# OSU-Bee-Lab/buzzdetect

Measured on AMD Instinct MI355X. Metric: yamnet_windows_per_s, higher is better.
Workload: dtype f32 (split-f16x3 MFMA products, f32 accumulate)

## Files before the change

buzzdetect_amd/csrc/bd_internal.h:

```cpp
#pragma once

#include <hip/hip_runtime.h>
#include <stdint.h>

#include <vector>

#include "../../include/buzzdetect_hip.h"

namespace bd {

constexpr int kMelNonZero = 461;

constexpr int kMelStart[BD_MEL_BANDS] = {
    5, 5, 6, 7, 9, 10, 11, 12, 13, 14, 16, 17, 18, 20, 21, 23, 25, 26, 28, 30, 32, 34, 36, 38, 40, 42, 44, 47, 49, 52, 54, 57,
    60, 63, 66, 69, 72, 76, 79, 83, 87, 90, 95, 99, 103, 108, 112, 117, 122, 127, 133, 138, 144, 150, 156, 162, 169, 176, 183,
    190, 198, 206, 214, 223};
constexpr int kMelLen[BD_MEL_BANDS] = {
    1, 2, 3, 3, 2, 2, 2, 2, 3, 3, 2, 3, 3, 3, 4, 3, 3, 4, 4, 4, 4, 4, 4, 4, 4, 5, 5, 5, 5, 5, 6, 6,
    6, 6, 6, 7, 7, 7, 8, 7, 8, 9, 8, 9, 9, 9, 10, 10, 11, 11, 11, 12, 12, 12, 13, 14, 14, 14, 15, 16, 16, 17, 17, 17};
constexpr int mel_offset(int band) {
    int o = 0;
    for (int m = 0; m < band; ++m) o += kMelLen[m];
    return o;
}
// ... 100 lines not shown
bool launch_l4_reg_f32(const float* in, float* out, int windows, const SepLayer& L4, const SepLayer& L5, hipStream_t stream);
bool launch_separable_chip(const float* in, float* out, int windows, const SepLayer* L, int nl, hipStream_t stream,
                           const SepLayer* next = nullptr, bool planes = false);
bool tail_supported(const SepLayer& L13, const SepLayer& L14);
bool launch_tail_pw13_dw14(const void* in, void* out, int windows, const SepLayer& L13, const SepLayer& L14, hipStream_t stream);
bool launch_tail_pw14_pool(const void* in, float* pooled, int windows, const SepLayer& L14, hipStream_t stream);
bool tail_f32_supported(const SepLayer& L13, const SepLayer& L14);
bool launch_tail_f32(const float* in, float* mid, float* pooled, int windows, const SepLayer& L13, const SepLayer& L14, hipStream_t stream,
                     int which);
bool launch_separable_chip_f32(const float* in, float* out, int windows, const SepLayer* L, int nl, hipStream_t stream,
                               const SepLayer* next, bool dw0_done);
bool launch_separable_mid_f32(const float* in, float* out, int windows, const SepLayer& L5, const SepLayer& L6, const SepLayer& L7,
                              hipStream_t stream);
bool launch_separable_mid(const float* in, float* out, int windows, const SepLayer& L5, const SepLayer& L6, const SepLayer& L7,
                          hipStream_t stream);
int launch_separable_run_next_dw(const float* a, float* b, int windows, const SepLayer* L, int max_layers, hipStream_t stream,
                                 bool planes = false);
bool launch_separable_fused_next_dw(const float* in, float* out, int windows, const SepLayer& L, const SepLayer& next,
                                    hipStream_t stream);
bool l4_window_planes_supported(const SepLayer& L3, const SepLayer& L4, const SepLayer& L5);
bool launch_l4_window_planes(const void* planes, const SepLayer& L3, const SepLayer& L4, const SepLayer& L5, float* out,
                             int windows, hipStream_t stream);
void launch_stem_reg(const float* logmel, int patch_step, const WindowMap& map, int w0, int windows, const float* c1_w,
                     const float* c1_b, const SepLayer& L2, const SepLayer& L3, float* out, hipStream_t stream);
void launch_stem_reg_planes(const float* logmel, int patch_step, const WindowMap& map, int w0, int windows, const float* c1_w,
                            const float* c1_b, const SepLayer& L2, const SepLayer& L3, float* out, hipStream_t stream);
void launch_stem_reg_f32(const float* logmel, int patch_step, const WindowMap& map, int w0, int windows, const float* c1_w,
                         const float* c1_b, const SepLayer& L2, const SepLayer& L3, float* out, hipStream_t stream);
void launch_stem4(const float* logmel, int patch_step, const WindowMap& map, int w0, int windows, const float* c1_w,
                  const float* c1_b,
// ... 8 lines not shown
```

buzzdetect_amd/csrc/engine.hip:

```cpp
#include <cmath>
#include <cstdio>
#include <cstdlib>
#include <cstring>
#include <unistd.h>
#include <memory>
#include <string>
#include <type_traits>
#include <utility>
#include <vector>

#include "bd_internal.h"

namespace {

thread_local std::string g_error;

int fail(int code, const std::string& msg) {
    g_error = msg;
    return code;
}

#define BD_HIP(expr)                                                                            \
    do {                                                                                        \
        hipError_t e_ = (expr);                                                                 \
        if (e_ != hipSuccess)                                                                   \
            return fail(BD_EHIP, std::string(#expr) + ": " + hipGetErrorString(e_));            \
    } while (0)

const int kLayerDefs[14][2] = {{2, 32},  {1, 64},  {2, 128}, {1, 128}, {2, 256}, {1, 256},  {2, 512},
                               {1, 512}, {1, 512}, {1, 512}, {1, 512}, {1, 512}, {2, 1024}, {1, 1024}};

constexpr int64_t kFloatsA = 98304;
constexpr int64_t kFloatsB = 49152;
constexpr int kDefaultGroup = 1024;
constexpr int kMaxGroup = 65536;
static_assert(kMaxGroup <= 1 << 17, "the tail launchers of pass_f16 / pass_f32 cover the largest pass");

inline int64_t align_up(int64_t v, int64_t a) { return (v + a - 1) / a * a; }

struct Event2 {
    hipEvent_t ev;
    int slot;
};

}

struct bd_engine {
    int device = 0;
    int n_classes = 0;
    int group_windows = kDefaultGroup;
    int pointwise_mode = 1;
// ... 808 lines not shown
    if (e->stem == 3 && e->separable != 0 && bd::l4_window_planes_supported(sep[1], sep[2], sep[3])) {
        stem(g, bd::launch_stem_reg_planes);
        if (!g.launch(7, [&] { return bd::launch_l4_window_planes(g.a, sep[1], sep[2], sep[3], g.b, g.gw, g.stream); }))
            return fail(BD_EHIP, "l4_window_kernel declined the planes of the stem");
    } else {
        if (e->stem != 0) {
            stem(g, e->stem == 3 ? bd::launch_stem_reg : bd::launch_stem4);
        } else {
            conv1(g);
            walk_layers(g, 0, false, 4);
        }
        if (e->separable == 0) return walk_layers(g, 2, false, -1);
        if (!g.launch(7, [&] { return bd::launch_separable_fused_next_dw(g.a, g.b, g.gw, sep[2], sep[3], g.stream); }))
            return walk_layers(g, 2, false, -1);
    }
    if (!(e->separable == 1 &&
          g.launch(13, [&] { return bd::launch_separable_mid(g.b, g.a, g.gw, sep[3], sep[4], sep[5], g.stream); }))) {
        pointwise(g, 3);
        if (!g.launch(11, [&] { return bd::launch_separable_fused_next_dw(g.a, g.b, g.gw, sep[4], sep[5], g.stream); }))
            return walk_layers(g, 4, false, -1);
        pointwise(g, 5);
    }
    const bool planes = bd::tail_supported(sep[11], sep[12]);
    if (!g.launch(23, [&] { return bd::launch_separable_run_next_dw(g.a, g.b, g.gw, &sep[6], 7, g.stream, planes); }))
        return walk_layers(g, 6, false, -1);
    if (!planes) return walk_layers(g, 11, true, -1);
    float* const pooled = g.emb ? g.emb : g.b;
    if (!g.launch(25, [&] { return bd::launch_tail_pw13_dw14(g.b, g.a, g.gw, sep[11], sep[12], g.stream); }) ||
        !g.launch(27, [&] { return bd::launch_tail_pw14_pool(g.a, pooled, g.gw, sep[12], g.stream); }))
        return fail(BD_EHIP, "septail.hip declined the planes of the on-chip run");
    return head(g, pooled);
}

int pass_f32(Group& g) {
    const bd_engine* e = g.e;
    const bd::SepLayer* sep = g.sep;
    stem(g, bd::launch_stem_reg_f32);
    if (e->separable == 0) return walk_layers(g, 2, false, -1);
    if (!g.launch(7, [&] { return bd::launch_l4_reg_f32(g.a, g.b, g.gw, sep[2], sep[3], g.stream); }))
        return walk_layers(g, 2, false, -1);
    bool dw8_done = false;
// ... 505 lines not shown
```

buzzdetect_amd/csrc/sepchip.hip:

```cpp
#include "bd_internal.h"

#include <cstdio>
#include <cstdlib>
#include <mutex>

namespace bd {

namespace {

typedef float f32x16 __attribute__((ext_vector_type(16)));
typedef float v2f __attribute__((ext_vector_type(2)));
typedef _Float16 f16x8 __attribute__((ext_vector_type(8)));

constexpr float kF16MaxChip = 65504.0f;

constexpr int kChipHalfBytes = 97 * 64;
constexpr int kChipSlotBytes = 2 * kChipHalfBytes;

constexpr int kChipMaxLayers = 5;
struct ChipChain {
    const float* dw_w[kChipMaxLayers];
    const float* dw_b[kChipMaxLayers];
    const _Float16* whi[kChipMaxLayers];
    const _Float16* wlo[kChipMaxLayers];
    const float* pw_u[kChipMaxLayers];
    const float* pw_b[kChipMaxLayers];
    const float* ndw_w;
};
template <typename T>
__device__ __forceinline__ const T* chain_ptr(int field, int li) {
    typedef const __attribute__((address_space(4))) unsigned long long* kptr;
    const kptr ka = (kptr)__builtin_amdgcn_kernarg_segment_ptr();
    return reinterpret_cast<const T*>(ka[field * kChipMaxLayers + li]);
}
static_assert(sizeof(ChipChain) == (6 * kChipMaxLayers + 1) * 8, "six tables of five pointers + one");

template <bool PLAIN, int NSLOT, bool TRACE = false, bool NDW = false, bool PLANES = false>
__global__ __launch_bounds__(512, 2) void sep_chip_kernel(const ChipChain ch, const float* X, float* Y, int nl,
                                                           long long M, unsigned* __restrict__ range_flag,
                                                           unsigned long long* __restrict__ dbg = nullptr, int tune = 0) {
    static_assert(NSLOT >= 9 && NSLOT <= 16, "ring size");
    constexpr int K = 512, KQ = K / 16;
    constexpr int NPEND = 16 - NSLOT;
    extern __shared__ __attribute__((aligned(16))) char sm[];
    const int tid = threadIdx.x;
    const int lane = tid & 63;
    const int wc = __builtin_amdgcn_readfirstlane(tid >> 6);
    const int frow = lane & 31, fh = lane >> 5;
    const long long m0 = (long long)blockIdx.x * 96;
    float rmax = 0.0f;
    int tsn = 0;
#define CHIP_TS()                                                                                         \
// ... 47 lines not shown
        char* const slot0 = sm + wc * kChipSlotBytes;                                                     \
        _Pragma("unroll") for (int rl = 0; rl < 48; ++rl) CHIP_PUT(slot0, rl, out0[rl])                   \
        if (wc + 8 < NSLOT) {                                                \
            char* const slot1 = sm + (wc + 8) * kChipSlotBytes;                                           \
            _Pragma("unroll") for (int rl = 0; rl < 48; ++rl) CHIP_PUT(slot1, rl, pend[rl])               \
        }                                                                                                 \
    }
#define CHIP_PUT(SLOT, RL, PK)                                                                            \
    {                                                                                                     \
        char* const p_ = (SLOT) + (wbl ^ ((((RL) >> 2) & 3) << 4)) + (RL) * 64;                           \
        *reinterpret_cast<unsigned short*>(p_) = (unsigned short)(PK);                                    \
        *reinterpret_cast<unsigned short*>(p_ + kChipHalfBytes) = (unsigned short)((PK) >> 16);           \
    }
#define CHIP_TAPS_RSRC(DW_W) __builtin_amdgcn_make_buffer_rsrc(const_cast<float*>(DW_W), 0, 10 * K * 4, 0x00020000)

    const long long rows_left = M - m0;
    const unsigned tile_bytes = (unsigned)(rows_left < 96 ? rows_left : 96) * (K * 4);
    {
        const __amdgpu_buffer_rsrc_t xrs = __builtin_amdgcn_make_buffer_rsrc(const_cast<float*>(X) + (size_t)m0 * K, 0, tile_bytes, 0x00020000);
        const __amdgpu_buffer_rsrc_t taps0 = CHIP_TAPS_RSRC(ch.dw_w[0]);
        const unsigned xo = (48u * fh * K) * 4 + c4;
#pragma unroll
        for (int j = 0; j < 2; ++j) {
            const int st = j ? wc + 8 : wc;
            v2f in2[6][4];
#pragma unroll
            for (int y = 0; y < 6; ++y)
#pragma unroll
                for (int x = 0; x < 4; ++x) {
                    in2[y][x].x = __builtin_bit_cast(float, __builtin_amdgcn_raw_buffer_load_b32(xrs, xo, ((4 * y + x) * K + 32 * st) * 4, 0));
                    in2[y][x].y = __builtin_bit_cast(float, __builtin_amdgcn_raw_buffer_load_b32(xrs, xo, ((24 + 4 * y + x) * K + 32 * st) * 4, 0));
                }
            if (j == 0) CHIP_DW(0, st, taps0)
            else CHIP_DW(1, st, taps0)
            CHIP_TS()
            __builtin_amdgcn_sched_barrier(0);
        }
        CHIP_PUBLISH()
    }

    for (int li = 0; li < nl; ++li) {
        const _Float16* const Wfhi = chain_ptr<_Float16>(2, li);
        const _Float16* const Wflo = chain_ptr<_Float16>(3, li);
        const __amdgpu_buffer_rsrc_t bhr = __builtin_amdgcn_make_buffer_rsrc(const_cast<_Float16*>(Wfhi), 0, K * K * 2, 0x00020000);
        const __amdgpu_buffer_rsrc_t blr = __builtin_amdgcn_make_buffer_rsrc(const_cast<_Float16*>(Wflo), 0, K * K * 2, 0x00020000);
        const int btile = wc * (KQ * 1024);
        constexpr int jstep = 8 * KQ * 1024;
        f16x8 bh0[2], bl0[2], bh1[2], bl1[2];
#define CHIP_LB(R, B, Q, J) B[J] = __builtin_bit_cast(f16x8, __builtin_amdgcn_raw_buffer_load_b128(R, lane16, btile + (J) * jstep + (Q) * 1024, 0));
#define CHIP_BLOAD(BH, BL, Q) { CHIP_LB(bhr, BH, Q, 0) CHIP_LB(blr, BL, Q, 0) CHIP_LB(bhr, BH, Q, 1) CHIP_LB(blr, BL, Q, 1) }
        CHIP_BLOAD(bh0, bl0, 0)
        __syncthreads();
        CHIP_TS()

        float zero;
        asm volatile("v_mov_b32 %0, 0" : "=v"(zero));
#pragma unroll
        for (int i = 0; i < 3; ++i)
#pragma unroll
            for (int j = 0; j < 2; ++j)
#pragma unroll
                for (int r = 0; r < 16; ++r) acc[i][j][r] = zero;
// ... 11 lines not shown
    }                                                                                                     \
    CHIP_MF(I, 0, AH, BH[0]) M3 CHIP_SB                                                                   \
    if constexpr (!PLAIN) {                                                                               \
        CHIP_MF(I, 1, AL, BH[1]) M4 CHIP_SB                                                               \
        CHIP_MF(I, 1, AH, BL[1]) M5 CHIP_SB                                                               \
    } else {                                                                                              \
        M4 M5                                                                                             \
    }                                                                                                     \
    CHIP_MF(I, 1, AH, BH[1]) M6 CHIP_SB
#define CHIP_STAGES(FROM, TO)                                                                             \
    if ((FROM) < (TO)) {                                                                                  \
        f16x8 ah0, al0, ah1, al1, ah2, al2;                                                               \
        const char* abase = sm + ((FROM) < NSLOT ? (FROM) : (FROM) - NSLOT) * kChipSlotBytes;             \
        CHIP_LAH(ah0, 0, 0) CHIP_LAL(al0, 0, 0) CHIP_LAH(ah1, 0, 1) CHIP_LAL(al1, 0, 1)                   \
        _Pragma("nounroll") for (int kk = (FROM); kk < (TO); ++kk) {                                      \
            const int q1 = 2 * kk + 1, q2 = 2 * kk + 2 < KQ ? 2 * kk + 2 : 0;      \
            const char* const anext = sm + (kk + 1 < (TO) ? (kk + 1 < NSLOT ? kk + 1 : kk + 1 - NSLOT) : (kk < NSLOT ? kk : kk - NSLOT)) * kChipSlotBytes; \
            CHIP_STEP(0, ah0, al0, bh0, bl0, CHIP_LB(bhr, bh1, q1, 0), CHIP_LB(blr, bl1, q1, 0), CHIP_LB(bhr, bh1, q1, 1),  \
                      CHIP_LB(blr, bl1, q1, 1), CHIP_LAH(ah2, 0, 2), CHIP_LAL(al2, 0, 2))                 \
            CHIP_STEP(1, ah1, al1, bh0, bl0, CHIP_LAH(ah0, 1, 0), CHIP_LAL(al0, 1, 0), CHIP_NOP, CHIP_NOP, CHIP_NOP, CHIP_NOP) \
            CHIP_STEP(2, ah2, al2, bh0, bl0, CHIP_LAH(ah1, 1, 1), CHIP_LAL(al1, 1, 1), CHIP_LB(blr, bl0, q2, 0),            \
                      CHIP_LB(bhr, bh0, q2, 0), CHIP_NOP, CHIP_LB(blr, bl0, q2, 1))                       \
            CHIP_STEP(0, ah0, al0, bh1, bl1, CHIP_LB(bhr, bh0, q2, 1), CHIP_LAH(ah2, 1, 2), CHIP_LAL(al2, 1, 2), CHIP_NOP, CHIP_NOP, CHIP_NOP) \
            abase = anext;          \
            CHIP_STEP(1, ah1, al1, bh1, bl1, CHIP_LAH(ah0, 0, 0), CHIP_LAL(al0, 0, 0), CHIP_NOP, CHIP_NOP, CHIP_NOP, CHIP_NOP) \
            CHIP_STEP(2, ah2, al2, bh1, bl1, CHIP_LAH(ah1, 0, 1), CHIP_LAL(al1, 0, 1), CHIP_NOP, CHIP_NOP, CHIP_NOP, CHIP_NOP) \
        }                                                                                                 \
    }
        CHIP_STAGES(0, NPEND)
        CHIP_TS()
        if constexpr (NPEND > 0) {
            __syncthreads();
            CHIP_TS()
            if (wc >= 8 - NPEND) {
                char* const slot = sm + (wc + 8 - NSLOT) * kChipSlotBytes;
                int wbl = wb0;
                asm volatile("" : "+v"(wbl));
#pragma unroll
                for (int rl = 0; rl < 48; ++rl) CHIP_PUT(slot, rl, pend[rl])
            }
        }
        CHIP_TS()
        if constexpr (NPEND > 0) __syncthreads();
        CHIP_TS()
        CHIP_STAGES(NPEND, 16)
        CHIP_TS()
#undef CHIP_STAGES
#undef CHIP_STEP
#undef CHIP_BLOAD
#undef CHIP_LB
#undef CHIP_LAH
#undef CHIP_LAL
#undef CHIP_MF
#undef CHIP_SB
#undef CHIP_NOP
        if (li + 1 == nl) break;

        const __amdgpu_buffer_rsrc_t taps = CHIP_TAPS_RSRC(chain_ptr<float>(0, li + 1));
        const __amdgpu_buffer_rsrc_t pur = __builtin_amdgcn_make_buffer_rsrc(const_cast<float*>(chain_ptr<float>(4, li)), 0, K * 4, 0x00020000);
        const __amdgpu_buffer_rsrc_t pbr = __builtin_amdgcn_make_buffer_rsrc(const_cast<float*>(chain_ptr<float>(5, li)), 0, K * 4, 0x00020000);
#pragma unroll
        for (int j = 0; j < 2; ++j) {
            const int st = j ? wc + 8 : wc;
            const float u = __builtin_bit_cast(float, __builtin_amdgcn_raw_buffer_load_b32(pur, c4, 128 * st, 0));
            const float b = __builtin_bit_cast(float, __builtin_amdgcn_raw_buffer_load_b32(pbr, c4, 128 * st, 0));
            float ev[12][4];
#pragma unroll
            for (int q = 0; q < 6; ++q)
#pragma unroll
                for (int x = 0; x < 4; ++x) {
                    const float a01 = fmaxf(fmaf(acc[q >> 2][j][4 * (q & 3) + x], u, b), 0.0f);
                    const float a23 = fmaxf(fmaf(acc[(q + 6) >> 2][j][4 * ((q + 6) & 3) + x], u, b), 0.0f);
                    const auto r = __builtin_amdgcn_permlane32_swap(__builtin_bit_cast(unsigned, a01),
                                                                    __builtin_bit_cast(unsigned, a23), false, false);
                    ev[2 * q][x] = __builtin_bit_cast(float, (unsigned)r[0]);
                    ev[2 * q + 1][x] = __builtin_bit_cast(float, (unsigned)r[1]);
                }
            v2f in2[6][4];
#pragma unroll
            for (int y = 0; y < 6; ++y)
#pragma unroll
                for (int x = 0; x < 4; ++x) in2[y][x] = v2f{ev[y][x], ev[6 + y][x]};
            if (j == 0) CHIP_DW(0, st, taps)
            else CHIP_DW(1, st, taps)
            CHIP_TS()
        }
        __syncthreads();
        CHIP_TS()
        CHIP_PUBLISH()
    }
#undef CHIP_DW
#undef CHIP_PUBLISH
#undef CHIP_TAPS_RSRC
#undef CHIP_PUT

    {
        const __amdgpu_buffer_rsrc_t pur = __builtin_amdgcn_make_buffer_rsrc(const_cast<float*>(chain_ptr<float>(4, nl - 1)), 0, K * 4, 0x00020000);
        const __amdgpu_buffer_rsrc_t pbr = __builtin_amdgcn_make_buffer_rsrc(const_cast<float*>(chain_ptr<float>(5, nl - 1)), 0, K * 4, 0x00020000);
        if constexpr (!NDW) {
            const __amdgpu_buffer_rsrc_t yrs = __builtin_amdgcn_make_buffer_rsrc(Y + (size_t)m0 * K, 0, tile_bytes, 0x00020000);
            const unsigned yo = (4u * fh * K) * 4 + c4;
#pragma unroll
            for (int j = 0; j < 2; ++j) {
                const int st = j ? wc + 8 : wc;
// ... 64 lines not shown
                                                                      ((6 * w + 2 * oy + ox) * K + 32 * st) * 4, 0);
                            }
                        }
                    }
            }
        }
    }
    if (range_flag && !(rmax <= kF16MaxChip)) *range_flag = 1u;
    if constexpr (TRACE) asm volatile("s_waitcnt vmcnt(0)" ::: "memory");
    CHIP_TS()
#undef CHIP_TS
}

constexpr int kMaxDevicesChip = 64;

template <bool PLAIN, bool NDW, bool PLANES = false>
void launch_chip(const float* in, float* out, const SepLayer* L, int nl, long long M, const float* ndw_w, hipStream_t stream) {
    ChipChain ch{};
    for (int i = 0; i < nl; ++i) {
        ch.dw_w[i] = dw_w_of(L[i]);
        ch.dw_b[i] = dw_b_of(L[i]);
        ch.whi[i] = static_cast<const _Float16*>(L[i].pw_fhi);
        ch.wlo[i] = static_cast<const _Float16*>(L[i].pw_flo);
        ch.pw_u[i] = L[i].pw_u;
        ch.pw_b[i] = L[i].pw_b;
    }
    ch.ndw_w = ndw_w;
    constexpr int NSLOT = 13;
    constexpr int lds = NSLOT * kChipSlotBytes;
    static_assert(lds <= 160 * 1024, "the ring must fit the CU's LDS");
    static std::once_flag once[kMaxDevicesChip];
    int dev = 0;
    (void)hipGetDevice(&dev);
    std::call_once(once[dev & (kMaxDevicesChip - 1)], [&] {
        (void)hipFuncSetAttribute(reinterpret_cast<const void*>(&sep_chip_kernel<PLAIN, NSLOT, false, NDW, PLANES>),
                                  hipFuncAttributeMaxDynamicSharedMemorySize, lds);
    });
    const long long tiles = (M + 95) / 96;
    int tune = 0;
#ifdef BD_KERNEL_TRACE
    if (const char* tn = getenv("BD_CHIP_TUNE")) tune = atoi(tn);
    const char* tr = getenv("BD_WS_TRACE");
    if (tr && tr[0] == '7' && !PLANES) {
        static unsigned long long* dbg = nullptr;
        static int shots = 0;
        if (!dbg) (void)hipMalloc(&dbg, 128 * 8);
        (void)hipFuncSetAttribute(reinterpret_cast<const void*>(&sep_chip_kernel<PLAIN, NSLOT, true, NDW>),
                                  hipFuncAttributeMaxDynamicSharedMemorySize, lds);
        (void)hipMemsetAsync(dbg, 0, 128 * 8, stream);
        hipLaunchKernelGGL((sep_chip_kernel<PLAIN, NSLOT, true, NDW>), dim3((unsigned)tiles), dim3(512), lds, stream, ch, in, out, nl,
                           M, L[0].range_flag, dbg, tune);
        (void)hipStreamSynchronize(stream);
        unsigned long long h[128];
        (void)hipMemcpy(h, dbg, sizeof(h), hipMemcpyDeviceToHost);
        if (++shots == 8)
            for (int w = 0; w < 2; ++w) {
                fprintf(stderr, "[trace] on-chip run of %d layers, wave %d: cycles between stamps (start | dw0 j0 j1 | per layer: B1, stages 0-2, B2, pend, "
                                "B3, stages 3-15, [dw j0, dw j1, B4] | stores):", nl, w ? 5 : 0);
                for (int i = 1; i < 64 && h[w * 64 + i]; ++i) fprintf(stderr, " %llu", h[w * 64 + i] - h[w * 64 + i - 1]);
                fprintf(stderr, "\n");
            }
        return;
    }
#endif
    hipLaunchKernelGGL((sep_chip_kernel<PLAIN, NSLOT, false, NDW, PLANES>), dim3((unsigned)tiles), dim3(512), lds, stream, ch, in, out, nl, M,
                       L[0].range_flag, (unsigned long long*)nullptr, tune);
}

}

bool launch_separable_chip(const float* in, float* out, int windows, const SepLayer* L, int nl, hipStream_t stream,
                           const SepLayer* next, bool planes) {
    if (planes && !next) return false;
    if (nl < 1 || nl > kChipMaxLayers) return false;
    for (int i = 0; i < nl; ++i)
        if (dw_b_of(L[i]) != dw_w_of(L[i]) + 9 * 512) return false;
    if (next && (dw_b_of(*next) != dw_w_of(*next) + 9 * 512 || next->cin != 512 || next->stride != 2 || in == out)) return false;
    const long long M = (long long)windows * 24;
    const float* nw = next ? dw_w_of(*next) : nullptr;
    if (planes) {
        if (L[0].pw_mode == 2) launch_chip<true, true, true>(in, out, L, nl, M, nw, stream);
        else launch_chip<false, true, true>(in, out, L, nl, M, nw, stream);
        return true;
    }
    if (L[0].pw_mode == 2) {
        if (next) launch_chip<true, true>(in, out, L, nl, M, nw, stream);
        else launch_chip<true, false>(in, out, L, nl, M, nw, stream);
    } else {
        if (next) launch_chip<false, true>(in, out, L, nl, M, nw, stream);
        else launch_chip<false, false>(in, out, L, nl, M, nw, stream);
    }
    return true;
}

}
```

buzzdetect_amd/csrc/sepmid.hip:

```cpp
#include "bd_internal.h"

#include <cstdio>
#include <cstdlib>
#include <mutex>
#include <type_traits>

namespace bd {

namespace {

typedef float f32x16 __attribute__((ext_vector_type(16)));
typedef float v2f __attribute__((ext_vector_type(2)));
typedef _Float16 f16x8 __attribute__((ext_vector_type(8)));

constexpr float kF16MaxMid = 65504.0f;
constexpr int kHalfA = 97 * 64;
constexpr int kSlotA = 2 * kHalfA;
constexpr int kHalf7 = 48 * 64;
constexpr int kSlot7 = 2 * kHalf7;
constexpr int kOffA7 = 8 * kSlotA;
constexpr int kMidLds = kOffA7 + 8 * kSlot7 + 1024;
static_assert(kMidLds <= 160 * 1024, "one workgroup per CU");

struct MidArgs {
    const _Float16 *w5h, *w5l, *w6h, *w6l, *w7h, *w7l;
    const float *u5, *b5, *u6, *b6, *u7, *b7;
    const float *dw6, *dw7;
};

#define MID_RSRC(P, BYTES) __builtin_amdgcn_make_buffer_rsrc(const_cast<void*>(static_cast<const void*>(P)), 0, (BYTES), 0x00020000)
#define MID_LD32(R, VOFF, SOFF) __builtin_bit_cast(float, __builtin_amdgcn_raw_buffer_load_b32(R, VOFF, SOFF, 0))
#define MID_LD128(R, VOFF, SOFF) __builtin_bit_cast(f16x8, __builtin_amdgcn_raw_buffer_load_b128(R, VOFF, SOFF, 0))

template <bool PLAIN, bool TRACE>
__global__ __launch_bounds__(512, 2) void sep_mid_kernel(const MidArgs a, const float* __restrict__ X, float* __restrict__ Y, int windows,
                                                          unsigned* __restrict__ range_flag, unsigned long long* __restrict__ dbg) {
    extern __shared__ __attribute__((aligned(16))) char sm[];
    const int tid = threadIdx.x, lane = tid & 63;
    const int wc = __builtin_amdgcn_readfirstlane(tid >> 6);
    const int frow = lane & 31, fh = lane >> 5;
    float rmax = 0.0f;
    int tsn = 0;
#define MID_TS()                                                                                          \
    if constexpr (TRACE) {                                                                                \
        if (blockIdx.x == 0 && lane == 0 && (wc == 0 || wc == 5) && tsn < 64)                             \
            dbg[(wc == 5 ? 64 : 0) + tsn] = __builtin_amdgcn_s_memtime();                                 \
        ++tsn;                                                                                            \
    }
    const int wb0 = fh * (48 * 64 + 64) + ((frow >> 3) << 4) + 2 * (frow & 7);
// ... 186 lines not shown
        MID_TS()
        if (win_next >= 0) fetch_window(win_next);
        {
            const __amdgpu_buffer_rsrc_t ur = MID_RSRC(a.u6, 1024), br = MID_RSRC(a.b6, 1024), tr = MID_RSRC(a.dw7, 10 * 256 * 4);
            const float u = MID_LD32(ur, c4, 128 * wc), b = MID_LD32(br, c4, 128 * wc);
            float wt[9];
#pragma unroll
            for (int t = 0; t < 9; ++t) wt[t] = MID_LD32(tr, c4, (t * 256 + 32 * wc) * 4);
            const float shift = MID_LD32(tr, c4, (9 * 256 + 32 * wc) * 4);
            float ev[12][4], lh[12], rh[12];
            MID_TILE_TO_MAP(acc, u, b, ev)
            MID_HALO(ev, lh, rh)
            int wbl = wb7;
            asm volatile("" : "+v"(wbl));
            char* const slot = sm + kOffA7 + wc * kSlot7;
            v2f in2[8][6];
            MID_ROW_PAIRS(ev, lh, rh, in2)
#pragma unroll
            for (int oy = 0; oy < 3; ++oy)
#pragma unroll
                for (int j = 0; j < 2; ++j) {
                    v2f sacc = {shift, shift};
#pragma unroll
                    for (int kh = 0; kh < 3; ++kh)
#pragma unroll
                        for (int kw = 0; kw < 3; ++kw)
                            sacc = __builtin_elementwise_fma(in2[1 + 2 * oy + kh][1 + 2 * j + kw], v2f{wt[kh * 3 + kw], wt[kh * 3 + kw]}, sacc);
#pragma unroll
                    for (int w = 0; w < 2; ++w) {
                        const int oyw = oy + 3 * w;
                        const float o = fmaxf(w ? sacc.y : sacc.x, 0.0f);
                        MID_SPLIT(o, pk)
                        char* const p_ = slot + (wbl ^ (((6 * HALF + oyw) & 3) << 4)) + (24 * HALF + 4 * oyw + j) * 64;
                        *reinterpret_cast<unsigned short*>(p_) = (unsigned short)pk;
                        *reinterpret_cast<unsigned short*>(p_ + kHalf7) = (unsigned short)(pk >> 16);
                    }
                }
        }
        if constexpr (LAST) {
#pragma unroll
            for (int q = 0; q < 2; ++q)
#pragma unroll
                for (int j = 0; j < 2; ++j) {
                    b7h[q][j] = MID_LD128(r7h, lane16, ((wc + 8 * j) * 16 + q) * 1024);
                    b7l[q][j] = MID_LD128(r7l, lane16, ((wc + 8 * j) * 16 + q) * 1024);
                }
        }
        __syncthreads();
        MID_TS()
    };
    auto layer7 = [&](auto nw_c, int win) {
        constexpr int NW = decltype(nw_c)::value;
// ... 34 lines not shown
            const float u = MID_LD32(ur, c4, 128 * (wc + 8 * j)), b = MID_LD32(br, c4, 128 * (wc + 8 * j));
#pragma unroll
            for (int i = 0; i < NW; ++i)
#pragma unroll
                for (int r = 0; r < (NW == 1 ? 12 : 16); ++r)
                    __builtin_amdgcn_raw_buffer_store_b32(__builtin_bit_cast(unsigned, fmaxf(fmaf(c7[i][j][r], u, b), 0.0f)), yr, yo,
                                                          ((32 * i + 8 * (r >> 2) + (r & 3)) * 512 + 32 * (wc + 8 * j)) * 4, 0);
        }
        MID_TS()
    };

    MID_TS()
    const int w_begin = (int)(((long long)blockIdx.x * windows) / gridDim.x);
    const int w_end = (int)(((long long)(blockIdx.x + 1) * windows) / gridDim.x);
    if (w_begin < w_end) fetch_window(w_begin);
    for (int win = w_begin; win < w_end; win += 2) {
        const bool two = win + 1 < w_end;
        if (two) {
            window_to_a7(std::integral_constant<int, 0>{}, std::false_type{}, win, win + 1);
            window_to_a7(std::integral_constant<int, 1>{}, std::true_type{}, win + 1, win + 2 < w_end ? win + 2 : -1);
            layer7(std::integral_constant<int, 2>{}, win);
        } else {
            window_to_a7(std::integral_constant<int, 0>{}, std::true_type{}, win, -1);
            layer7(std::integral_constant<int, 1>{}, win);
        }
    }
    if (range_flag && !(rmax <= kF16MaxMid)) *range_flag = 1u;
#undef MID_TS
#undef MID_PUT
#undef MID_SPLIT
#undef MID_MMA
#undef MID_TILE_TO_MAP
#undef MID_HALO
}

template <bool PLAIN>
void launch_mid(const float* in, float* out, int windows, const SepLayer& L5, const SepLayer& L6, const SepLayer& L7, hipStream_t stream) {
    MidArgs a{};
    a.w5h = static_cast<const _Float16*>(L5.pw_fhi);
    a.w5l = static_cast<const _Float16*>(L5.pw_flo);
    a.w6h = static_cast<const _Float16*>(L6.pw_fhi);
    a.w6l = static_cast<const _Float16*>(L6.pw_flo);
    a.w7h = static_cast<const _Float16*>(L7.pw_fhi);
    a.w7l = static_cast<const _Float16*>(L7.pw_flo);
    a.u5 = L5.pw_u; a.b5 = L5.pw_b;
    a.u6 = L6.pw_u; a.b6 = L6.pw_b;
    a.u7 = L7.pw_u; a.b7 = L7.pw_b;
    a.dw6 = dw_w_of(L6);
    a.dw7 = dw_w_of(L7);
    static std::once_flag once[64];
    int dev = 0;
    (void)hipGetDevice(&dev);
    std::call_once(once[dev & 63], [&] {
        (void)hipFuncSetAttribute(reinterpret_cast<const void*>(&sep_mid_kernel<PLAIN, false>), hipFuncAttributeMaxDynamicSharedMemorySize, kMidLds);
    });
    int grid = cu_count();
    if (grid > windows) grid = windows;
#ifdef BD_KERNEL_TRACE
    const char* tr = getenv("BD_WS_TRACE");
    if (tr && tr[0] == '8') {
        static unsigned long long* dbg = nullptr;
        static int shots = 0;
        if (!dbg) (void)hipMalloc(&dbg, 128 * 8);
        (void)hipFuncSetAttribute(reinterpret_cast<const void*>(&sep_mid_kernel<PLAIN, true>), hipFuncAttributeMaxDynamicSharedMemorySize, kMidLds);
        (void)hipMemsetAsync(dbg, 0, 128 * 8, stream);
        hipLaunchKernelGGL((sep_mid_kernel<PLAIN, true>), dim3(grid), dim3(512), kMidLds, stream, a, in, out, windows, L5.range_flag, dbg);
        (void)hipStreamSynchronize(stream);
        unsigned long long h[128];
        (void)hipMemcpy(h, dbg, sizeof(h), hipMemcpyDeviceToHost);
        if (++shots == 8)
            for (int w = 0; w < 2; ++w) {
                fprintf(stderr, "[trace] mid run, wave %d: cycles between stamps (per window: A5+B1, K5, dw6+Bx, publish+B2, K6, dw7+B3; per pair: K7, stores):", w ? 5 : 0);
                for (int i = 1; i < 64 && h[w * 64 + i]; ++i) fprintf(stderr, " %llu", h[w * 64 + i] - h[w * 64 + i - 1]);
                fprintf(stderr, "\n");
            }
        return;
    }
#endif
    hipLaunchKernelGGL((sep_mid_kernel<PLAIN, false>), dim3(grid), dim3(512), kMidLds, stream, a, in, out, windows, L5.range_flag,
                       (unsigned long long*)nullptr);
}

}

bool launch_separable_mid(const float* in, float* out, int windows, const SepLayer& L5, const SepLayer& L6, const SepLayer& L7,
                          hipStream_t stream) {
    if (windows <= 0 || in == out) return false;
    if (L5.cin != 128 || L5.cout != 256 || L5.h_out != 12 || L5.w_out != 8 || L6.cin != 256 || L6.cout != 256 || L6.stride != 1 ||
        L6.h_out != 12 || L6.w_out != 8 || L7.cin != 256 || L7.cout != 512 || L7.stride != 2 || L7.h_out != 6 || L7.w_out != 4)
        return false;
    if (L5.pw_mode == 0 || L6.pw_mode != L5.pw_mode || L7.pw_mode != L5.pw_mode) return false;
    if (dw_b_of(L6) != dw_w_of(L6) + 9 * 256 || dw_b_of(L7) != dw_w_of(L7) + 9 * 256) return false;
    if (L5.pw_mode == 2) launch_mid<true>(in, out, windows, L5, L6, L7, stream);
    else launch_mid<false>(in, out, windows, L5, L6, L7, stream);
    return true;
}

}
```

Before: 1.975 million.

## Move layer-7 pointwise from mid kernel into chip kernel via depthwise-7 planes

The middle kernel can now stop after depthwise-7 and store its split-f16 output as per-window planes in global memory. The chip kernel gains a PW7 mode that loads those planes straight into LDS, runs the K=256 pointwise-7 MFMA loop, and then continues with layers 8-12 in the same launch. The goal is to rebalance work between the two kernels and avoid writing and re-reading the f32 layer-7 output. In exchange the code path is more complex, the mid kernel processes one window per iteration instead of pairs, and the chip kernel takes on more registers and work.

```diff
diff --git a/buzzdetect_amd/csrc/bd_internal.h b/buzzdetect_amd/csrc/bd_internal.h
--- a/buzzdetect_amd/csrc/bd_internal.h
+++ b/buzzdetect_amd/csrc/bd_internal.h
@@ -138,6 +138,13 @@
                               hipStream_t stream);
 bool launch_separable_mid(const float* in, float* out, int windows, const SepLayer& L5, const SepLayer& L6, const SepLayer& L7,
                           hipStream_t stream);
+constexpr int kDw7PlaneBytes = 8 * 2 * 24 * 32 * 2;
+bool separable_mid_planes_supported(const SepLayer& L5, const SepLayer& L6, const SepLayer& L7);
+bool launch_separable_mid_planes(const float* in, void* out, int windows, const SepLayer& L5, const SepLayer& L6, const SepLayer& L7,
+                                 hipStream_t stream);
+bool separable_chip_pw7_supported(const SepLayer& L7, const SepLayer* L, int nl, const SepLayer& next, int windows);
+bool launch_separable_chip_pw7(const void* in, float* out, int windows, const SepLayer& L7, const SepLayer* L, int nl,
+                               const SepLayer& next, hipStream_t stream);
 int launch_separable_run_next_dw(const float* a, float* b, int windows, const SepLayer* L, int max_layers, hipStream_t stream,
                                  bool planes = false);
 bool launch_separable_fused_next_dw(const float* in, float* out, int windows, const SepLayer& L, const SepLayer& next,
diff --git a/buzzdetect_amd/csrc/engine.hip b/buzzdetect_amd/csrc/engine.hip
--- a/buzzdetect_amd/csrc/engine.hip
+++ b/buzzdetect_amd/csrc/engine.hip
@@ -35,6 +35,7 @@
 constexpr int kDefaultGroup = 1024;
 constexpr int kMaxGroup = 65536;
 static_assert(kMaxGroup <= 1 << 17, "the tail launchers of pass_f16 / pass_f32 cover the largest pass");
+static_assert(bd::kDw7PlaneBytes <= kFloatsA * 4, "the depthwise-7 planes of the middle run fit buffer a");
 
 inline int64_t align_up(int64_t v, int64_t a) { return (v + a - 1) / a * a; }
 
@@ -873,17 +874,25 @@
         if (!g.launch(7, [&] { return bd::launch_separable_fused_next_dw(g.a, g.b, g.gw, sep[2], sep[3], g.stream); }))
             return walk_layers(g, 2, false, -1);
     }
-    if (!(e->separable == 1 &&
-          g.launch(13, [&] { return bd::launch_separable_mid(g.b, g.a, g.gw, sep[3], sep[4], sep[5], g.stream); }))) {
-        pointwise(g, 3);
-        if (!g.launch(11, [&] { return bd::launch_separable_fused_next_dw(g.a, g.b, g.gw, sep[4], sep[5], g.stream); }))
-            return walk_layers(g, 4, false, -1);
-        pointwise(g, 5);
-    }
     const bool planes = bd::tail_supported(sep[11], sep[12]);
-    if (!g.launch(23, [&] { return bd::launch_separable_run_next_dw(g.a, g.b, g.gw, &sep[6], 7, g.stream, planes); }))
-        return walk_layers(g, 6, false, -1);
-    if (!planes) return walk_layers(g, 11, true, -1);
+    if (e->separable == 1 && planes && bd::separable_mid_planes_supported(sep[3], sep[4], sep[5]) &&
+        bd::separable_chip_pw7_supported(sep[5], &sep[6], 5, sep[11], g.gw)) {
+        if (!g.launch(13, [&] { return bd::launch_separable_mid_planes(g.b, g.a, g.gw, sep[3], sep[4], sep[5], g.stream); }))
+            return fail(BD_EHIP, "sep_mid_kernel declined the depthwise-7 planes");
+        if (!g.launch(23, [&] { return bd::launch_separable_chip_pw7(g.a, g.b, g.gw, sep[5], &sep[6], 5, sep[11], g.stream); }))
+            return fail(BD_EHIP, "sep_chip_kernel declined the planes of the middle run");
+    } else {
+        if (!(e->separable == 1 &&
+              g.launch(13, [&] { return bd::launch_separable_mid(g.b, g.a, g.gw, sep[3], sep[4], sep[5], g.stream); }))) {
+            pointwise(g, 3);
+            if (!g.launch(11, [&] { return bd::launch_separable_fused_next_dw(g.a, g.b, g.gw, sep[4], sep[5], g.stream); }))
+                return walk_layers(g, 4, false, -1);
+            pointwise(g, 5);
+        }
+        if (!g.launch(23, [&] { return bd::launch_separable_run_next_dw(g.a, g.b, g.gw, &sep[6], 7, g.stream, planes); }))
+            return walk_layers(g, 6, false, -1);
+        if (!planes) return walk_layers(g, 11, true, -1);
+    }
     float* const pooled = g.emb ? g.emb : g.b;
     if (!g.launch(25, [&] { return bd::launch_tail_pw13_dw14(g.b, g.a, g.gw, sep[11], sep[12], g.stream); }) ||
         !g.launch(27, [&] { return bd::launch_tail_pw14_pool(g.a, pooled, g.gw, sep[12], g.stream); }))
diff --git a/buzzdetect_amd/csrc/sepchip.hip b/buzzdetect_amd/csrc/sepchip.hip
--- a/buzzdetect_amd/csrc/sepchip.hip
+++ b/buzzdetect_amd/csrc/sepchip.hip
@@ -26,6 +26,8 @@
     const float* pw_u[kChipMaxLayers];
     const float* pw_b[kChipMaxLayers];
     const float* ndw_w;
+    const _Float16 *w7hi, *w7lo;
+    const float *u7, *b7;
 };
 template <typename T>
 __device__ __forceinline__ const T* chain_ptr(int field, int li) {
@@ -33,9 +35,9 @@
     const kptr ka = (kptr)__builtin_amdgcn_kernarg_segment_ptr();
     return reinterpret_cast<const T*>(ka[field * kChipMaxLayers + li]);
 }
-static_assert(sizeof(ChipChain) == (6 * kChipMaxLayers + 1) * 8, "six tables of five pointers + one");
-
-template <bool PLAIN, int NSLOT, bool TRACE = false, bool NDW = false, bool PLANES = false>
+static_assert(sizeof(ChipChain) == (6 * kChipMaxLayers + 5) * 8, "six tables of five pointers + five");
+
+template <bool PLAIN, int NSLOT, bool TRACE = false, bool NDW = false, bool PLANES = false, bool PW7 = false>
 __global__ __launch_bounds__(512, 2) void sep_chip_kernel(const ChipChain ch, const float* X, float* Y, int nl,
                                                            long long M, unsigned* __restrict__ range_flag,
                                                            unsigned long long* __restrict__ dbg = nullptr, int tune = 0) {
@@ -113,38 +115,15 @@
     }
 #define CHIP_TAPS_RSRC(DW_W) __builtin_amdgcn_make_buffer_rsrc(const_cast<float*>(DW_W), 0, 10 * K * 4, 0x00020000)
 
-    const long long rows_left = M - m0;
-    const unsigned tile_bytes = (unsigned)(rows_left < 96 ? rows_left : 96) * (K * 4);
-    {
-        const __amdgpu_buffer_rsrc_t xrs = __builtin_amdgcn_make_buffer_rsrc(const_cast<float*>(X) + (size_t)m0 * K, 0, tile_bytes, 0x00020000);
-        const __amdgpu_buffer_rsrc_t taps0 = CHIP_TAPS_RSRC(ch.dw_w[0]);
-        const unsigned xo = (48u * fh * K) * 4 + c4;
-#pragma unroll
-        for (int j = 0; j < 2; ++j) {
-            const int st = j ? wc + 8 : wc;
-            v2f in2[6][4];
-#pragma unroll
-            for (int y = 0; y < 6; ++y)
-#pragma unroll
-                for (int x = 0; x < 4; ++x) {
-                    in2[y][x].x = __builtin_bit_cast(float, __builtin_amdgcn_raw_buffer_load_b32(xrs, xo, ((4 * y + x) * K + 32 * st) * 4, 0));
-                    in2[y][x].y = __builtin_bit_cast(float, __builtin_amdgcn_raw_buffer_load_b32(xrs, xo, ((24 + 4 * y + x) * K + 32 * st) * 4, 0));
-                }
-            if (j == 0) CHIP_DW(0, st, taps0)
-            else CHIP_DW(1, st, taps0)
-            CHIP_TS()
-            __builtin_amdgcn_sched_barrier(0);
-        }
-        CHIP_PUBLISH()
-    }
-
-    for (int li = 0; li < nl; ++li) {
-        const _Float16* const Wfhi = chain_ptr<_Float16>(2, li);
-        const _Float16* const Wflo = chain_ptr<_Float16>(3, li);
-        const __amdgpu_buffer_rsrc_t bhr = __builtin_amdgcn_make_buffer_rsrc(const_cast<_Float16*>(Wfhi), 0, K * K * 2, 0x00020000);
-        const __amdgpu_buffer_rsrc_t blr = __builtin_amdgcn_make_buffer_rsrc(const_cast<_Float16*>(Wflo), 0, K * K * 2, 0x00020000);
-        const int btile = wc * (KQ * 1024);
-        constexpr int jstep = 8 * KQ * 1024;
+    auto k_loop = [&](auto kq_c, const _Float16* const Wfhi, const _Float16* const Wflo) __attribute__((always_inline)) {
+        constexpr int KQL = decltype(kq_c)::value;
+        constexpr int NS = KQL / 2;
+        constexpr int NP = NS > NSLOT ? NS - NSLOT : 0;
+        static_assert(NP == 0 || NP == NPEND, "a layer of K = 512 or one that fits the ring");
+        const __amdgpu_buffer_rsrc_t bhr = __builtin_amdgcn_make_buffer_rsrc(const_cast<_Float16*>(Wfhi), 0, 16 * KQL * K * 2, 0x00020000);
+        const __amdgpu_buffer_rsrc_t blr = __builtin_amdgcn_make_buffer_rsrc(const_cast<_Float16*>(Wflo), 0, 16 * KQL * K * 2, 0x00020000);
+        const int btile = wc * (KQL * 1024);
+        constexpr int jstep = 8 * KQL * 1024;
         f16x8 bh0[2], bl0[2], bh1[2], bl1[2];
 #define CHIP_LB(R, B, Q, J) B[J] = __builtin_bit_cast(f16x8, __builtin_amdgcn_raw_buffer_load_b128(R, lane16, btile + (J) * jstep + (Q) * 1024, 0));
 #define CHIP_BLOAD(BH, BL, Q) { CHIP_LB(bhr, BH, Q, 0) CHIP_LB(blr, BL, Q, 0) CHIP_LB(bhr, BH, Q, 1) CHIP_LB(blr, BL, Q, 1) }
@@ -186,7 +165,7 @@
         const char* abase = sm + ((FROM) < NSLOT ? (FROM) : (FROM) - NSLOT) * kChipSlotBytes;             \
         CHIP_LAH(ah0, 0, 0) CHIP_LAL(al0, 0, 0) CHIP_LAH(ah1, 0, 1) CHIP_LAL(al1, 0, 1)                   \
         _Pragma("nounroll") for (int kk = (FROM); kk < (TO); ++kk) {                                      \
-            const int q1 = 2 * kk + 1, q2 = 2 * kk + 2 < KQ ? 2 * kk + 2 : 0;      \
+            const int q1 = 2 * kk + 1, q2 = 2 * kk + 2 < KQL ? 2 * kk + 2 : 0;     \
             const char* const anext = sm + (kk + 1 < (TO) ? (kk + 1 < NSLOT ? kk + 1 : kk + 1 - NSLOT) : (kk < NSLOT ? kk : kk - NSLOT)) * kChipSlotBytes; \
             CHIP_STEP(0, ah0, al0, bh0, bl0, CHIP_LB(bhr, bh1, q1, 0), CHIP_LB(blr, bl1, q1, 0), CHIP_LB(bhr, bh1, q1, 1),  \
                       CHIP_LB(blr, bl1, q1, 1), CHIP_LAH(ah2, 0, 2), CHIP_LAL(al2, 0, 2))                 \
@@ -199,9 +178,9 @@
             CHIP_STEP(2, ah2, al2, bh1, bl1, CHIP_LAH(ah1, 0, 1), CHIP_LAL(al1, 0, 1), CHIP_NOP, CHIP_NOP, CHIP_NOP, CHIP_NOP) \
         }                                                                                                 \
     }
-        CHIP_STAGES(0, NPEND)
-        CHIP_TS()
-        if constexpr (NPEND > 0) {
+        CHIP_STAGES(0, NP)
+        CHIP_TS()
+        if constexpr (NP > 0) {
             __syncthreads();
             CHIP_TS()
             if (wc >= 8 - NPEND) {
@@ -213,9 +192,9 @@
             }
         }
         CHIP_TS()
-        if constexpr (NPEND > 0) __syncthreads();
-        CHIP_TS()
-        CHIP_STAGES(NPEND, 16)
+        if constexpr (NP > 0) __syncthreads();
+        CHIP_TS()
+        CHIP_STAGES(NP, NS)
         CHIP_TS()
 #undef CHIP_STAGES
 #undef CHIP_STEP
@@ -226,11 +205,12 @@
 #undef CHIP_MF
 #undef CHIP_SB
 #undef CHIP_NOP
-        if (li + 1 == nl) break;
-
-        const __amdgpu_buffer_rsrc_t taps = CHIP_TAPS_RSRC(chain_ptr<float>(0, li + 1));
-        const __amdgpu_buffer_rsrc_t pur = __builtin_amdgcn_make_buffer_rsrc(const_cast<float*>(chain_ptr<float>(4, li)), 0, K * 4, 0x00020000);
-        const __amdgpu_buffer_rsrc_t pbr = __builtin_amdgcn_make_buffer_rsrc(const_cast<float*>(chain_ptr<float>(5, li)), 0, K * 4, 0x00020000);
+    };
+
+    auto next_layer = [&](const float* const taps_w, const float* const pu, const float* const pb) __attribute__((always_inline)) {
+        const __amdgpu_buffer_rsrc_t taps = CHIP_TAPS_RSRC(taps_w);
+        const __amdgpu_buffer_rsrc_t pur = __builtin_amdgcn_make_buffer_rsrc(const_cast<float*>(pu), 0, K * 4, 0x00020000);
+        const __amdgpu_buffer_rsrc_t pbr = __builtin_amdgcn_make_buffer_rsrc(const_cast<float*>(pb), 0, K * 4, 0x00020000);
 #pragma unroll
         for (int j = 0; j < 2; ++j) {
             const int st = j ? wc + 8 : wc;
@@ -260,6 +240,64 @@
         __syncthreads();
         CHIP_TS()
         CHIP_PUBLISH()
+    };
+
+    const long long rows_left = M - m0;
+    const unsigned tile_bytes = (unsigned)(rows_left < 96 ? rows_left : 96) * (K * 4);
+    if constexpr (PW7) {
+        const long long w0 = m0 / 24, wleft = M / 24 - w0;
+        const __amdgpu_buffer_rsrc_t pr = __builtin_amdgcn_make_buffer_rsrc(
+            const_cast<char*>(reinterpret_cast<const char*>(X)) + (size_t)w0 * kDw7PlaneBytes, 0,
+            (unsigned)(wleft < 4 ? wleft : 4) * kDw7PlaneBytes, 0x00020000);
+        constexpr int kPieces = 8 * kChipSlotBytes / 1024;
+        static_assert(kPieces * 1024 == 8 * kChipSlotBytes && 8 * kChipSlotBytes <= NSLOT * kChipSlotBytes, "whole pieces");
+#pragma unroll
+        for (int t = 0; t < (kPieces + 7) / 8; ++t) {
+            const int n = 8 * t + wc;
+            if (n >= kPieces) break;
+            const int c = 64 * n + lane;
+            const int s = c / (kChipSlotBytes / 16), cs = c - s * (kChipSlotBytes / 16);
+            const int h = cs >= kChipHalfBytes / 16 ? 1 : 0;
+            const int o = (cs - h * (kChipHalfBytes / 16)) * 16;
+            const bool skew = o >= 48 * 64 && o < 49 * 64;
+            const int rho = o < 48 * 64 ? o >> 6 : (o - 64) >> 6;
+            const int p = (o >> 4) & 3, w = rho / 24;
+            const unsigned src = (unsigned)(w * kDw7PlaneBytes + s * (kDw7PlaneBytes / 8) + h * (kDw7PlaneBytes / 16) +
+                                            (rho - 24 * w) * 64 + ((p ^ ((rho >> 2) & 3)) << 4));
+            const unsigned off = skew || (PLAIN && h) ? 0x7ffffff0u : src;
+            __builtin_amdgcn_raw_ptr_buffer_load_lds(pr, (__attribute__((address_space(3))) void*)(sm + n * 1024), 16, off, 0, 0, 0);
+        }
+        asm volatile("s_waitcnt vmcnt(0)" ::: "memory");
+        CHIP_TS()
+        k_loop(std::integral_constant<int, 16>{}, ch.w7hi, ch.w7lo);
+        next_layer(ch.dw_w[0], ch.u7, ch.b7);
+    } else {
+        const __amdgpu_buffer_rsrc_t xrs = __builtin_amdgcn_make_buffer_rsrc(const_cast<float*>(X) + (size_t)m0 * K, 0, tile_bytes, 0x00020000);
+        const __amdgpu_buffer_rsrc_t taps0 = CHIP_TAPS_RSRC(ch.dw_w[0]);
+        const unsigned xo = (48u * fh * K) * 4 + c4;
+#pragma unroll
+        for (int j = 0; j < 2; ++j) {
+            const int st = j ? wc + 8 : wc;
+            v2f in2[6][4];
+#pragma unroll
+            for (int y = 0; y < 6; ++y)
+#pragma unroll
+                for (int x = 0; x < 4; ++x) {
+                    in2[y][x].x = __builtin_bit_cast(float, __builtin_amdgcn_raw_buffer_load_b32(xrs, xo, ((4 * y + x) * K + 32 * st) * 4, 0));
+                    in2[y][x].y = __builtin_bit_cast(float, __builtin_amdgcn_raw_buffer_load_b32(xrs, xo, ((24 + 4 * y + x) * K + 32 * st) * 4, 0));
+                }
+            if (j == 0) CHIP_DW(0, st, taps0)
+            else CHIP_DW(1, st, taps0)
+            CHIP_TS()
+            __builtin_amdgcn_sched_barrier(0);
+        }
+        CHIP_PUBLISH()
+    }
+
+    for (int li = 0; li < nl; ++li) {
+        k_loop(std::integral_constant<int, KQ>{}, chain_ptr<_Float16>(2, li), chain_ptr<_Float16>(3, li));
+        if (li + 1 == nl) break;
+        next_layer(chain_ptr<float>(0, li + 1), chain_ptr<float>(4, li), chain_ptr<float>(5, li));
     }
 #undef CHIP_DW
 #undef CHIP_PUBLISH
@@ -354,9 +392,16 @@
 
 constexpr int kMaxDevicesChip = 64;
 
-template <bool PLAIN, bool NDW, bool PLANES = false>
-void launch_chip(const float* in, float* out, const SepLayer* L, int nl, long long M, const float* ndw_w, hipStream_t stream) {
+template <bool PLAIN, bool NDW, bool PLANES = false, bool PW7 = false>
+void launch_chip(const float* in, float* out, const SepLayer* L, int nl, long long M, const float* ndw_w, hipStream_t stream,
+                 const SepLayer* L7 = nullptr) {
     ChipChain ch{};
+    if (L7) {
+        ch.w7hi = static_cast<const _Float16*>(L7->pw_fhi);
+        ch.w7lo = static_cast<const _Float16*>(L7->pw_flo);
+        ch.u7 = L7->pw_u;
+        ch.b7 = L7->pw_b;
+    }
     for (int i = 0; i < nl; ++i) {
         ch.dw_w[i] = dw_w_of(L[i]);
         ch.dw_b[i] = dw_b_of(L[i]);
@@ -373,7 +418,7 @@
     int dev = 0;
     (void)hipGetDevice(&dev);
     std::call_once(once[dev & (kMaxDevicesChip - 1)], [&] {
-        (void)hipFuncSetAttribute(reinterpret_cast<const void*>(&sep_chip_kernel<PLAIN, NSLOT, false, NDW, PLANES>),
+        (void)hipFuncSetAttribute(reinterpret_cast<const void*>(&sep_chip_kernel<PLAIN, NSLOT, false, NDW, PLANES, PW7>),
                                   hipFuncAttributeMaxDynamicSharedMemorySize, lds);
     });
     const long long tiles = (M + 95) / 96;
@@ -381,29 +426,30 @@
 #ifdef BD_KERNEL_TRACE
     if (const char* tn = getenv("BD_CHIP_TUNE")) tune = atoi(tn);
     const char* tr = getenv("BD_WS_TRACE");
-    if (tr && tr[0] == '7' && !PLANES) {
+    if (tr && tr[0] == '7') {
         static unsigned long long* dbg = nullptr;
         static int shots = 0;
         if (!dbg) (void)hipMalloc(&dbg, 128 * 8);
-        (void)hipFuncSetAttribute(reinterpret_cast<const void*>(&sep_chip_kernel<PLAIN, NSLOT, true, NDW>),
+        (void)hipFuncSetAttribute(reinterpret_cast<const void*>(&sep_chip_kernel<PLAIN, NSLOT, true, NDW, PLANES, PW7>),
                                   hipFuncAttributeMaxDynamicSharedMemorySize, lds);
         (void)hipMemsetAsync(dbg, 0, 128 * 8, stream);
-        hipLaunchKernelGGL((sep_chip_kernel<PLAIN, NSLOT, true, NDW>), dim3((unsigned)tiles), dim3(512), lds, stream, ch, in, out, nl,
+        hipLaunchKernelGGL((sep_chip_kernel<PLAIN, NSLOT, true, NDW, PLANES, PW7>), dim3((unsigned)tiles), dim3(512), lds, stream, ch, in, out, nl,
                            M, L[0].range_flag, dbg, tune);
         (void)hipStreamSynchronize(stream);
         unsigned long long h[128];
         (void)hipMemcpy(h, dbg, sizeof(h), hipMemcpyDeviceToHost);
         if (++shots == 8)
             for (int w = 0; w < 2; ++w) {
-                fprintf(stderr, "[trace] on-chip run of %d layers, wave %d: cycles between stamps (start | dw0 j0 j1 | per layer: B1, stages 0-2, B2, pend, "
-                                "B3, stages 3-15, [dw j0, dw j1, B4] | stores):", nl, w ? 5 : 0);
+                fprintf(stderr, "[trace] on-chip run of %d layers%s, wave %d: cycles between stamps (start | %s | per layer: B1, stages 0-2, B2, pend, "
+                                "B3, stages 3-15, [dw j0, dw j1, B4] | stores):", nl, PW7 ? " + pointwise 7" : "", w ? 5 : 0,
+                        PW7 ? "DMA, B1, -, -, -, stages 0-7, dw j0, dw j1, B4" : "dw0 j0 j1");
                 for (int i = 1; i < 64 && h[w * 64 + i]; ++i) fprintf(stderr, " %llu", h[w * 64 + i] - h[w * 64 + i - 1]);
                 fprintf(stderr, "\n");
             }
         return;
     }
 #endif
-    hipLaunchKernelGGL((sep_chip_kernel<PLAIN, NSLOT, false, NDW, PLANES>), dim3((unsigned)tiles), dim3(512), lds, stream, ch, in, out, nl, M,
+    hipLaunchKernelGGL((sep_chip_kernel<PLAIN, NSLOT, false, NDW, PLANES, PW7>), dim3((unsigned)tiles), dim3(512), lds, stream, ch, in, out, nl, M,
                        L[0].range_flag, (unsigned long long*)nullptr, tune);
 }
 
@@ -433,4 +479,25 @@
     return true;
 }
 
-}
+bool separable_chip_pw7_supported(const SepLayer& L7, const SepLayer* L, int nl, const SepLayer& next, int windows) {
+    if (windows <= 0 || (long long)windows * 24 >= (1LL << 31) || nl < 1 || nl > kChipMaxLayers) return false;
+    if (L7.cin != 256 || L7.cout != 512 || L7.h_out != 6 || L7.w_out != 4 || L7.pw_mode == 0 || !L7.pw_fhi || !L7.pw_flo)
+        return false;
+    for (int i = 0; i < nl; ++i)
+        if (L[i].stride != 1 || L[i].cin != 512 || L[i].cout != 512 || L[i].h_out != 6 || L[i].w_out != 4 ||
+            L[i].pw_mode != L7.pw_mode || dw_b_of(L[i]) != dw_w_of(L[i]) + 9 * 512)
+            return false;
+    return next.stride == 2 && next.cin == 512 && dw_b_of(next) == dw_w_of(next) + 9 * 512;
+}
+
+bool launch_separable_chip_pw7(const void* in, float* out, int windows, const SepLayer& L7, const SepLayer* L, int nl,
+                               const SepLayer& next, hipStream_t stream) {
+    if (!separable_chip_pw7_supported(L7, L, nl, next, windows) || in == out) return false;
+    const float* const X = static_cast<const float*>(in);
+    const long long M = (long long)windows * 24;
+    if (L7.pw_mode == 2) launch_chip<true, true, true, true>(X, out, L, nl, M, dw_w_of(next), stream, &L7);
+    else launch_chip<false, true, true, true>(X, out, L, nl, M, dw_w_of(next), stream, &L7);
+    return true;
+}
+
+}
diff --git a/buzzdetect_amd/csrc/sepmid.hip b/buzzdetect_amd/csrc/sepmid.hip
--- a/buzzdetect_amd/csrc/sepmid.hip
+++ b/buzzdetect_amd/csrc/sepmid.hip
@@ -21,6 +21,9 @@
 constexpr int kOffA7 = 8 * kSlotA;
 constexpr int kMidLds = kOffA7 + 8 * kSlot7 + 1024;
 static_assert(kMidLds <= 160 * 1024, "one workgroup per CU");
+constexpr int kStage7 = kDw7PlaneBytes / 8;
+constexpr int kMidLdsDw7 = kOffA7 + 8 * kStage7;
+static_assert(kStage7 == 2 * 24 * 64, "[hi, lo][24 rows][32 channels] f16");
 
 struct MidArgs {
     const _Float16 *w5h, *w5l, *w6h, *w6l, *w7h, *w7l;
@@ -32,7 +35,7 @@
 #define MID_LD32(R, VOFF, SOFF) __builtin_bit_cast(float, __builtin_amdgcn_raw_buffer_load_b32(R, VOFF, SOFF, 0))
 #define MID_LD128(R, VOFF, SOFF) __builtin_bit_cast(f16x8, __builtin_amdgcn_raw_buffer_load_b128(R, VOFF, SOFF, 0))
 
-template <bool PLAIN, bool TRACE>
+template <bool PLAIN, bool TRACE, bool DW7OUT = false>
 __global__ __launch_bounds__(512, 2) void sep_mid_kernel(const MidArgs a, const float* __restrict__ X, float* __restrict__ Y, int windows,
                                                           unsigned* __restrict__ range_flag, unsigned long long* __restrict__ dbg) {
     extern __shared__ __attribute__((aligned(16))) char sm[];
@@ -249,6 +252,7 @@
             int wbl = wb7;
             asm volatile("" : "+v"(wbl));
             char* const slot = sm + kOffA7 + wc * kSlot7;
+            char* const stg = sm + kOffA7 + wc * kStage7;
             v2f in2[8][6];
             MID_ROW_PAIRS(ev, lh, rh, in2)
 #pragma unroll
@@ -266,11 +270,29 @@
                         const int oyw = oy + 3 * w;
                         const float o = fmaxf(w ? sacc.y : sacc.x, 0.0f);
                         MID_SPLIT(o, pk)
-                        char* const p_ = slot + (wbl ^ (((6 * HALF + oyw) & 3) << 4)) + (24 * HALF + 4 * oyw + j) * 64;
-                        *reinterpret_cast<unsigned short*>(p_) = (unsigned short)pk;
-                        *reinterpret_cast<unsigned short*>(p_ + kHalf7) = (unsigned short)(pk >> 16);
+                        if constexpr (DW7OUT) {
+                            char* const p_ = stg + (4 * oyw + 2 * fh + j) * 64 + 2 * frow;
+                            *reinterpret_cast<unsigned short*>(p_) = (unsigned short)pk;
+                            if constexpr (!PLAIN) *reinterpret_cast<unsigned short*>(p_ + kStage7 / 2) = (unsigned short)(pk >> 16);
+                        } else {
+                            char* const p_ = slot + (wbl ^ (((6 * HALF + oyw) & 3) << 4)) + (24 * HALF + 4 * oyw + j) * 64;
+                            *reinterpret_cast<unsigned short*>(p_) = (unsigned short)pk;
+                            *reinterpret_cast<unsigned short*>(p_ + kHalf7) = (unsigned short)(pk >> 16);
+                        }
                     }
                 }
+            if constexpr (DW7OUT) {
+                typedef __attribute__((address_space(1))) char* gchar;
+                typedef float v4f __attribute__((ext_vector_type(4)));
+                asm volatile("" ::: "memory");
+                const gchar dst = (gchar)Y + (size_t)win * kDw7PlaneBytes + wc * kStage7 + lane * 16;
+#pragma unroll
+                for (int t = 0; t < 3; ++t) {
+                    if (PLAIN && (t == 2 || (t == 1 && lane >= 32))) continue;
+                    const v4f v = *reinterpret_cast<const v4f*>(stg + t * 1024 + lane * 16);
+                    asm volatile("global_store_dwordx4 %0, %1, off\n\ts_nop 2" : : "v"(dst + t * 1024), "v"(v) : "memory");
+                }
+            }
         }
         if constexpr (LAST) {
 #pragma unroll
@@ -335,7 +357,10 @@
     const int w_begin = (int)(((long long)blockIdx.x * windows) / gridDim.x);
     const int w_end = (int)(((long long)(blockIdx.x + 1) * windows) / gridDim.x);
     if (w_begin < w_end) fetch_window(w_begin);
-    for (int win = w_begin; win < w_end; win += 2) {
+    if constexpr (DW7OUT) {
+        for (int win = w_begin; win < w_end; ++win)
+            window_to_a7(std::integral_constant<int, 0>{}, std::false_type{}, win, win + 1 < w_end ? win + 1 : -1);
+    } else for (int win = w_begin; win < w_end; win += 2) {
         const bool two = win + 1 < w_end;
         if (two) {
             window_to_a7(std::integral_constant<int, 0>{}, std::false_type{}, win, win + 1);
@@ -355,8 +380,9 @@
 #undef MID_HALO
 }
 
-template <bool PLAIN>
+template <bool PLAIN, bool DW7OUT>
 void launch_mid(const float* in, float* out, int windows, const SepLayer& L5, const SepLayer& L6, const SepLayer& L7, hipStream_t stream) {
+    constexpr int lds = DW7OUT ? kMidLdsDw7 : kMidLds;
     MidArgs a{};
     a.w5h = static_cast<const _Float16*>(L5.pw_fhi);
     a.w5l = static_cast<const _Float16*>(L5.pw_flo);
@@ -373,7 +399,7 @@
     int dev = 0;
     (void)hipGetDevice(&dev);
     std::call_once(once[dev & 63], [&] {
-        (void)hipFuncSetAttribute(reinterpret_cast<const void*>(&sep_mid_kernel<PLAIN, false>), hipFuncAttributeMaxDynamicSharedMemorySize, kMidLds);
+        (void)hipFuncSetAttribute(reinterpret_cast<const void*>(&sep_mid_kernel<PLAIN, false, DW7OUT>), hipFuncAttributeMaxDynamicSharedMemorySize, lds);
     });
     int grid = cu_count();
     if (grid > windows) grid = windows;
@@ -383,38 +409,55 @@
         static unsigned long long* dbg = nullptr;
         static int shots = 0;
         if (!dbg) (void)hipMalloc(&dbg, 128 * 8);
-        (void)hipFuncSetAttribute(reinterpret_cast<const void*>(&sep_mid_kernel<PLAIN, true>), hipFuncAttributeMaxDynamicSharedMemorySize, kMidLds);
+        (void)hipFuncSetAttribute(reinterpret_cast<const void*>(&sep_mid_kernel<PLAIN, true, DW7OUT>), hipFuncAttributeMaxDynamicSharedMemorySize, lds);
         (void)hipMemsetAsync(dbg, 0, 128 * 8, stream);
-        hipLaunchKernelGGL((sep_mid_kernel<PLAIN, true>), dim3(grid), dim3(512), kMidLds, stream, a, in, out, windows, L5.range_flag, dbg);
+        hipLaunchKernelGGL((sep_mid_kernel<PLAIN, true, DW7OUT>), dim3(grid), dim3(512), lds, stream, a, in, out, windows, L5.range_flag, dbg);
         (void)hipStreamSynchronize(stream);
         unsigned long long h[128];
         (void)hipMemcpy(h, dbg, sizeof(h), hipMemcpyDeviceToHost);
         if (++shots == 8)
             for (int w = 0; w < 2; ++w) {
-                fprintf(stderr, "[trace] mid run, wave %d: cycles between stamps (per window: A5+B1, K5, dw6+Bx, publish+B2, K6, dw7+B3; per pair: K7, stores):", w ? 5 : 0);
+                fprintf(stderr, "[trace] mid run, wave %d: cycles between stamps (per window: A5+B1, K5, dw6+Bx, publish+B2, K6, %s):", w ? 5 : 0,
+                        DW7OUT ? "dw7 + its planes stored" : "dw7+B3; per pair: K7, stores");
                 for (int i = 1; i < 64 && h[w * 64 + i]; ++i) fprintf(stderr, " %llu", h[w * 64 + i] - h[w * 64 + i - 1]);
                 fprintf(stderr, "\n");
             }
         return;
     }
 #endif
-    hipLaunchKernelGGL((sep_mid_kernel<PLAIN, false>), dim3(grid), dim3(512), kMidLds, stream, a, in, out, windows, L5.range_flag,
+    hipLaunchKernelGGL((sep_mid_kernel<PLAIN, false, DW7OUT>), dim3(grid), dim3(512), lds, stream, a, in, out, windows, L5.range_flag,
                        (unsigned long long*)nullptr);
 }
 
 }
 
-bool launch_separable_mid(const float* in, float* out, int windows, const SepLayer& L5, const SepLayer& L6, const SepLayer& L7,
-                          hipStream_t stream) {
-    if (windows <= 0 || in == out) return false;
+namespace {
+bool mid_shapes_ok(const SepLayer& L5, const SepLayer& L6, const SepLayer& L7) {
     if (L5.cin != 128 || L5.cout != 256 || L5.h_out != 12 || L5.w_out != 8 || L6.cin != 256 || L6.cout != 256 || L6.stride != 1 ||
         L6.h_out != 12 || L6.w_out != 8 || L7.cin != 256 || L7.cout != 512 || L7.stride != 2 || L7.h_out != 6 || L7.w_out != 4)
         return false;
     if (L5.pw_mode == 0 || L6.pw_mode != L5.pw_mode || L7.pw_mode != L5.pw_mode) return false;
-    if (dw_b_of(L6) != dw_w_of(L6) + 9 * 256 || dw_b_of(L7) != dw_w_of(L7) + 9 * 256) return false;
-    if (L5.pw_mode == 2) launch_mid<true>(in, out, windows, L5, L6, L7, stream);
-    else launch_mid<false>(in, out, windows, L5, L6, L7, stream);
+    return dw_b_of(L6) == dw_w_of(L6) + 9 * 256 && dw_b_of(L7) == dw_w_of(L7) + 9 * 256;
+}
+}
+
+bool launch_separable_mid(const float* in, float* out, int windows, const SepLayer& L5, const SepLayer& L6, const SepLayer& L7,
+                          hipStream_t stream) {
+    if (windows <= 0 || in == out || !mid_shapes_ok(L5, L6, L7)) return false;
+    if (L5.pw_mode == 2) launch_mid<true, false>(in, out, windows, L5, L6, L7, stream);
+    else launch_mid<false, false>(in, out, windows, L5, L6, L7, stream);
     return true;
 }
 
-}
+bool separable_mid_planes_supported(const SepLayer& L5, const SepLayer& L6, const SepLayer& L7) { return mid_shapes_ok(L5, L6, L7); }
+
+bool launch_separable_mid_planes(const float* in, void* out, int windows, const SepLayer& L5, const SepLayer& L6, const SepLayer& L7,
+                                 hipStream_t stream) {
+    if (windows <= 0 || in == out || !mid_shapes_ok(L5, L6, L7)) return false;
+    float* const Y = static_cast<float*>(out);
+    if (L5.pw_mode == 2) launch_mid<true, true>(in, Y, windows, L5, L6, L7, stream);
+    else launch_mid<false, true>(in, Y, windows, L5, L6, L7, stream);
+    return true;
+}
+
+}
```

Result: faster. 2.026 million, median of 6 (+2.6%).
